# SeanNaren/deepspeech.pytorch

Hardware: NVIDIA H100
Metric: utterances/sec (train step, 161x1000 spectrogram) (higher is better)
Workload: dtype fp16-operands(rnn)+tf32(conv/fc)

## Files before the change

### deepspeech.pytorch_b200/csrc/common.cuh

```cuda
#pragma once
#include <cuda_runtime.h>
#include <stdint.h>
#include <stdio.h>
#include <string.h>
#include <atomic>

#include "../../include/ds2_b200.h"

namespace ds2 {

void set_error(const char* fmt, ...);
extern std::atomic<long long> g_launches;
int precision();
inline bool tensor_core_mode() { return precision() != DS2_PREC_FP32; }
inline bool f16_gemm_mode() { return precision() == DS2_PREC_F16; }

inline cudaStream_t as_stream(void* s) { return reinterpret_cast<cudaStream_t>(s); }

inline int current_device() {
  int d = 0;
  (void)cudaGetDevice(&d);
  return d & 63;
}
struct DeviceOnce {
// ... 62 lines not shown

#ifdef __CUDACC__
__device__ __forceinline__ float sigmoidf_(float x) { return 1.0f / (1.0f + expf(-x)); }

__device__ __forceinline__ float warp_sum(float v) {
#pragma unroll
  for (int o = 16; o > 0; o >>= 1) v += __shfl_xor_sync(0xffffffffu, v, o);
  return v;
}
__device__ __forceinline__ double warp_sum_d(double v) {
#pragma unroll
  for (int o = 16; o > 0; o >>= 1) v += __shfl_xor_sync(0xffffffffu, v, o);
  return v;
}
#endif

int gemm_simt(int transA, int transB, int M, int N, int K, float alpha, const float* A, int lda, const float* B,
              int ldb, float beta, float* C, int ldc, cudaStream_t st, void* ws = nullptr, size_t ws_bytes = 0);
size_t gemm_simt_workspace_bytes(int M, int N, int K);
int gemm_tc(int transA, int transB, int M, int N, int K, float alpha, const float* A, int lda, const float* B,
            int ldb, float beta, float* C, int ldc, void* ws, size_t ws_bytes, cudaStream_t st);
size_t gemm_tc_workspace_bytes(int transA, int transB, int M, int N, int K);
int gemm_tc_f16(int M, int N, int K, float alpha, const void* A16, int lda, const void* B16, int ldb, float beta,
                float* C, int ldc, const float* alpha_dev, cudaStream_t st);
int f32_to_f16_rows(int rows, int cols, const float* in, size_t ld_in, void* out, size_t ld_out, const float* scale_dev,
                    cudaStream_t st);
int f32_to_f16_transpose(int rows, int cols, const float* in, size_t ld_in, void* out, size_t ld_out, void* outT,
                         size_t ld_outT, const float* scale_dev, cudaStream_t st);
int pow2_scale_for(int rows, int cols, const float* x, size_t ld, unsigned int* absmax_ws, float* scale, int top,
                   cudaStream_t st);

int bn_rows_fwd(int rows, int F, const float* x, const float* gamma, const float* beta, float* rmean, float* rvar,
                int training, float momentum, float eps, float* y, float* xhat, float* mean_invstd ,
                double* ws_sums , cudaStream_t st);
int bn_rows_reapply(int rows, int F, const float* x, const float* gamma, const float* beta,
                    const float* mean_invstd, float* y, float* xhat, cudaStream_t st);
int transpose(int R, int C, const float* in, float* out, cudaStream_t st);
int transpose_strided(int R, int C, const float* in, size_t ldi, float* out, size_t ldo, cudaStream_t st);
int bn_rows_bwd(int rows, int F, const float* xhat, const float* gamma, const float* mean_invstd, const float* dy,
                float* dx, float* dgamma, float* dbeta, double* ws_sums , cudaStream_t st);

}
```

### deepspeech.pytorch_b200/csrc/gemm_tc.cu

```cuda
#include <stdio.h>

#include "common.cuh"
#include "tc_common.cuh"

namespace ds2 {

typedef CUresult (*EncodeTiledFn)(CUtensorMap*, CUtensorMapDataType, cuuint32_t, void*, const cuuint64_t*,
                                  const cuuint64_t*, const cuuint32_t*, const cuuint32_t*, CUtensorMapInterleave,
                                  CUtensorMapSwizzle, CUtensorMapL2promotion, CUtensorMapFloatOOBfill);
static EncodeTiledFn g_encode = nullptr;
static constexpr CUtensorMapDataType g_tmap_dtype = CU_TENSOR_MAP_DATA_TYPE_TFLOAT32;

static int load_encode() {
  if (g_encode) return DS2_OK;
  void* fn = nullptr;
  cudaDriverEntryPointQueryResult q;
  DS2_CHECK_CUDA(cudaGetDriverEntryPoint("cuTensorMapEncodeTiled", &fn, cudaEnableDefault, &q));
  if (!fn || q != cudaDriverEntryPointSuccess) {
    set_error("cuTensorMapEncodeTiled not available from the driver");
    return DS2_ERR_CUDA;
  }
  g_encode = reinterpret_cast<EncodeTiledFn>(fn);
  return DS2_OK;
}

static int make_tmap_2d_sw(CUtensorMap* out, const float* base, int rows, int cols, int ld, int box_rows, int box_cols,
                           CUtensorMapSwizzle sw);
int make_tmap_2d(CUtensorMap* out, const float* base, int rows, int cols, int ld, int box_rows, int box_cols) {
  return make_tmap_2d_sw(out, base, rows, cols, ld, box_rows, box_cols, CU_TENSOR_MAP_SWIZZLE_128B);
}
static int make_tmap_2d_sw(CUtensorMap* out, const float* base, int rows, int cols, int ld, int box_rows, int box_cols,
                           CUtensorMapSwizzle sw) {
  int rc = load_encode();
  if (rc) return rc;
  cuuint64_t gdim[2] = {(cuuint64_t)cols, (cuuint64_t)rows};
  cuuint64_t gstr[1] = {(cuuint64_t)ld * sizeof(float)};
  cuuint32_t box[2] = {(cuuint32_t)box_cols, (cuuint32_t)box_rows};
  cuuint32_t estr[2] = {1, 1};
  CUresult r = g_encode(out, g_tmap_dtype, 2, const_cast<float*>(base), gdim, gstr, box, estr,
                        CU_TENSOR_MAP_INTERLEAVE_NONE, sw, CU_TENSOR_MAP_L2_PROMOTION_L2_256B,
                        CU_TENSOR_MAP_FLOAT_OOB_FILL_NONE);
  if (r != CUDA_SUCCESS) {
    set_error("cuTensorMapEncodeTiled(2d rows=%d cols=%d ld=%d box=%dx%d base=%p) failed: %d", rows, cols, ld,
              box_rows, box_cols, (const void*)base, (int)r);
    return DS2_ERR_CUDA;
  }
  return DS2_OK;
}

static int make_tmap_3d_sw(CUtensorMap* out, const float* base, int d0, int d1, int d2, size_t stride1, size_t stride2,
                           int box0, int box1, int box2, CUtensorMapSwizzle sw);
int make_tmap_3d(CUtensorMap* out, const float* base, int d0, int d1, int d2, size_t stride1, size_t stride2,
                 int box0, int box1, int box2) {
  return make_tmap_3d_sw(out, base, d0, d1, d2, stride1, stride2, box0, box1, box2, CU_TENSOR_MAP_SWIZZLE_128B);
}
static int make_tmap_3d_sw(CUtensorMap* out, const float* base, int d0, int d1, int d2, size_t stride1, size_t stride2,
                           int box0, int box1, int box2, CUtensorMapSwizzle sw) {
  int rc = load_encode();
  if (rc) return rc;
  cuuint64_t gdim[3] = {(cuuint64_t)d0, (cuuint64_t)d1, (cuuint64_t)d2};
  cuuint64_t gstr[2] = {(cuuint64_t)stride1 * sizeof(float), (cuuint64_t)stride2 * sizeof(float)};
  cuuint32_t box[3] = {(cuuint32_t)box0, (cuuint32_t)box1, (cuuint32_t)box2};
// ... 53 lines not shown
  cuuint32_t box[3] = {(cuuint32_t)box0, (cuuint32_t)box1, (cuuint32_t)box2};
  cuuint32_t estr[3] = {1, 1, 1};
  CUresult r = g_encode(out, CU_TENSOR_MAP_DATA_TYPE_FLOAT16, (cuuint32_t)rank, const_cast<void*>(base), gdim, gstr,
                        box, estr, CU_TENSOR_MAP_INTERLEAVE_NONE, CU_TENSOR_MAP_SWIZZLE_128B,
                        CU_TENSOR_MAP_L2_PROMOTION_L2_256B, CU_TENSOR_MAP_FLOAT_OOB_FILL_NONE);
  if (r != CUDA_SUCCESS) {
    set_error("cuTensorMapEncodeTiled(f16 rank %d dims %d,%d,%d box %d,%d,%d) failed: %d", rank, d0, d1, d2, box0, box1,
              box2, (int)r);
    return DS2_ERR_CUDA;
  }
  return DS2_OK;
}

namespace gtc {
constexpr int BM = 128, BK = 32, THREADS = 384;
constexpr int PRODUCER_REGS = 40, MMA_REGS = 232;
template <int BN>
struct Cfg {
  static constexpr int STAGES = BN == 256 ? 4 : 6;
  static constexpr int A_BYTES = BM * 128, B_BYTES = BN * 128, STAGE_BYTES = A_BYTES + B_BYTES;
  static constexpr int SMEM_BYTES = STAGES * STAGE_BYTES + 1024  + 256 ;
};
static_assert(Cfg<256>::SMEM_BYTES <= 227 * 1024 && Cfg<128>::SMEM_BYTES <= 227 * 1024, "shared memory");
}

template <bool F16, int BN>
__global__ void __launch_bounds__(gtc::THREADS, 1)
gemm_tc_kernel(const __grid_constant__ CUtensorMap tmA, const __grid_constant__ CUtensorMap tmB, int M, int N, int K,
               float alpha, float beta, float* __restrict__ C, int ldc, const float* __restrict__ alpha_dev) {
  using namespace gtc;
  using namespace tc;
  constexpr int STAGES = Cfg<BN>::STAGES, A_BYTES = Cfg<BN>::A_BYTES, STAGE_BYTES = Cfg<BN>::STAGE_BYTES;
  constexpr int BK = F16 ? 2 * gtc::BK : gtc::BK;
  if (alpha_dev) alpha *= __ldg(alpha_dev);
  extern __shared__ uint8_t smem_raw[];
  uint8_t* smem = smem_raw + ((1024u - (smem_u32(smem_raw) & 1023u)) & 1023u);
  uint64_t* full = reinterpret_cast<uint64_t*>(smem + STAGES * STAGE_BYTES);
  uint64_t* empty = full + STAGES;
  const int warp = threadIdx.x / 32, lane = threadIdx.x % 32;
  const int m0 = blockIdx.y * BM, n0 = blockIdx.x * BN;
  const int nk = (K + BK - 1) / BK;

  if (warp == 0 && lane == 0) {
    tma_prefetch_desc(&tmA);
    tma_prefetch_desc(&tmB);
    for (int i = 0; i < STAGES; ++i) { mbar_init(&full[i], 1); mbar_init(&empty[i], 2); }
// ... 49 lines not shown
        float2 o = make_float2(alpha * acc[4 * i + 2 * hh], alpha * acc[4 * i + 2 * hh + 1]);
        if (vec_ok && col + 1 < N) {
          float2* cp2 = reinterpret_cast<float2*>(crow + col);
          if (beta != 0.f) {
            const float2 old = *cp2;
            o.x = fmaf(beta, old.x, o.x);
            o.y = fmaf(beta, old.y, o.y);
          }
          *cp2 = o;
        } else {
#pragma unroll
          for (int j = 0; j < 2; ++j) {
            if (col + j >= N) break;
            float v = j ? o.y : o.x;
            if (beta != 0.f) v = fmaf(beta, crow[col + j], v);
            crow[col + j] = v;
          }
        }
      }
    }
  }
}

__global__ void transpose_strided_kernel(int R, int C, const float* __restrict__ in, size_t ldi,
                                         float* __restrict__ out, size_t ldo) {
  __shared__ float tile[32][33];
  int c = blockIdx.x * 32 + threadIdx.x, r0 = blockIdx.y * 32;
  for (int j = threadIdx.y; j < 32; j += 8)
    if (r0 + j < R && c < C) tile[j][threadIdx.x] = in[(size_t)(r0 + j) * ldi + c];
  __syncthreads();
  int r = r0 + threadIdx.x, c0 = blockIdx.x * 32;
  for (int j = threadIdx.y; j < 32; j += 8)
    if (c0 + j < C && r < R) out[(size_t)(c0 + j) * ldo + r] = tile[threadIdx.x][j];
}

int transpose_strided(int R, int C, const float* in, size_t ldi, float* out, size_t ldo, cudaStream_t st) {
  DS2_LAUNCH(transpose_strided_kernel, dim3(cdiv(C, 32), cdiv(R, 32)), dim3(32, 8), 0, st, R, C, in, ldi, out, ldo);
  return DS2_OK;
}
int transpose(int R, int C, const float* in, float* out, cudaStream_t st) {
  return transpose_strided(R, C, in, (size_t)C, out, (size_t)R, st);
}

static inline size_t k4(int K) { return (size_t)((K + 3) / 4 * 4); }

struct GemmTcWs { float *At, *Bt; };
static size_t gemm_tc_ws_carve(int transA, int transB, int M, int N, int K, void* base, GemmTcWs& w) {
  size_t off = 0;
  w.At = transA ? carve<float>(base, off, (size_t)M * k4(K) * 4) : nullptr;
  w.Bt = transB ? nullptr : carve<float>(base, off, (size_t)N * k4(K) * 4);
  return off;
}

size_t gemm_tc_workspace_bytes(int transA, int transB, int M, int N, int K) {
  GemmTcWs w;
  return gemm_tc_ws_carve(transA, transB, M, N, K, nullptr, w);
}

static bool tc_eligible(int M, int N, int K) { return K >= 32 && M >= 32 && N >= 16 && (long long)M * N * K >= (1 << 18); }

static int tile_n(int N) { return N > 128 ? 256 : 128; }

template <bool F16, int BN>
static int launch_gemm_tc(const CUtensorMap& tmA, const CUtensorMap& tmB, int M, int N, int K, float alpha, float beta,
                          float* C, int ldc, cudaStream_t st, const float* alpha_dev) {
  auto kern = gemm_tc_kernel<F16, BN>;
  constexpr int smem = gtc::Cfg<BN>::SMEM_BYTES;
  static DeviceOnce attr_once;
  if (attr_once.first()) {
    DS2_CHECK_CUDA(cudaFuncSetAttribute(kern, cudaFuncAttributeMaxDynamicSharedMemorySize, smem));
    attr_once.done();
  }
  dim3 grid(cdiv(N, BN), cdiv(M, gtc::BM));
  DS2_LAUNCH(kern, grid, gtc::THREADS, smem, st, tmA, tmB, M, N, K, alpha, beta, C, ldc, alpha_dev);
  return DS2_OK;
}

template <bool F16>
static int launch_gemm_tc(const CUtensorMap& tmA, const CUtensorMap& tmB, int M, int N, int K, float alpha, float beta,
                          float* C, int ldc, cudaStream_t st, const float* alpha_dev = nullptr) {
  if (tile_n(N) == 256) return launch_gemm_tc<F16, 256>(tmA, tmB, M, N, K, alpha, beta, C, ldc, st, alpha_dev);
  return launch_gemm_tc<F16, 128>(tmA, tmB, M, N, K, alpha, beta, C, ldc, st, alpha_dev);
}

int gemm_tc(int transA, int transB, int M, int N, int K, float alpha, const float* A, int lda, const float* B,
            int ldb, float beta, float* C, int ldc, void* ws, size_t ws_bytes, cudaStream_t st) {
  if (!tc_eligible(M, N, K)) return 1;
  GemmTcWs W;
  if (gemm_tc_ws_carve(transA, transB, M, N, K, ws, W) > (ws ? ws_bytes : 0)) return 1;
  const float* Ak = A;
  int ldak = lda;
  if (transA) {
    int rc = transpose_strided(K, M, A, (size_t)lda, W.At, k4(K), st);
    if (rc) return rc;
    Ak = W.At;
    ldak = (int)k4(K);
  }
  const float* Bk = B;
  int ldbk = ldb;
  if (!transB) {
    int rc = transpose_strided(K, N, B, (size_t)ldb, W.Bt, k4(K), st);
    if (rc) return rc;
    Bk = W.Bt;
    ldbk = (int)k4(K);
  }
  if ((ldak & 3) || (ldbk & 3) || (reinterpret_cast<uintptr_t>(Ak) & 15) || (reinterpret_cast<uintptr_t>(Bk) & 15))
    return 1;
  CUtensorMap tmA, tmB;
  int rc = make_tmap_2d(&tmA, Ak, M, K, ldak, gtc::BM, gtc::BK);
  if (rc) return rc;
  rc = make_tmap_2d(&tmB, Bk, N, K, ldbk, tile_n(N), gtc::BK);
  if (rc) return rc;
  return launch_gemm_tc<false>(tmA, tmB, M, N, K, alpha, beta, C, ldc, st);
}

int gemm_tc_f16(int M, int N, int K, float alpha, const void* A16, int lda, const void* B16, int ldb, float beta,
                float* C, int ldc, const float* alpha_dev, cudaStream_t st) {
  if (!tc_eligible(M, N, K) || M < 128) return 1;
  if ((lda & 7) || (ldb & 7) || (reinterpret_cast<uintptr_t>(A16) & 15) || (reinterpret_cast<uintptr_t>(B16) & 15)) return 1;
  CUtensorMap tmA, tmB;
  int rc = make_tmap_f16(&tmA, A16, 2, K, M, 1, (size_t)lda, 0, 64, gtc::BM, 1);
  if (rc) return rc;
  rc = make_tmap_f16(&tmB, B16, 2, K, N, 1, (size_t)ldb, 0, 64, tile_n(N), 1);
  if (rc) return rc;
  return launch_gemm_tc<true>(tmA, tmB, M, N, K, alpha, beta, C, ldc, st, alpha_dev);
}

}
```

### deepspeech.pytorch_b200/csrc/rnn_layer.cu

```cuda
#include <cuda_fp16.h>

#include <mutex>
#include <unordered_set>

#include "common.cuh"
#include "rnn_cells.cuh"
#include "rnn_common.cuh"

namespace ds2 {

constexpr int UT = 8;
constexpr int KC = 64;

template <int RNN>
__global__ void __launch_bounds__(32 * UT) rnn_step_fwd_kernel(SeqArgs a, int step) {
  constexpr int G = num_gates(RNN);
  __shared__ float hs[32][KC + 1];
  __shared__ float ws[G * UT][KC + 1];
  const int d = blockIdx.y, T = a.T, B = a.B, H = a.H, D = a.D;
  const int t = d == 0 ? step : T - 1 - step;
  const int tp = d == 0 ? t - 1 : t + 1;
  const bool tp_in = tp >= 0 && tp < T;
  const int lane = threadIdx.x, uy = threadIdx.y, tid = uy * 32 + lane;
  const int u0 = blockIdx.x * UT, u = u0 + uy;
// ... 490 lines not shown
  if (f16 && side && d->deferred_dw) {
    rc = side_fork(st, side);
    if (rc) return rc;
    gst = side;
  }
  if (f16) {
    rc = f32_to_f16_transpose(TB, In, xin, (size_t)In, nullptr, 0, W.x16T, (size_t)TB, nullptr, gst);
    if (rc) return rc;
    for (int dir = 0; dir < D; ++dir) {
      rc = f32_to_f16_transpose(TB, H, R.hseq + (size_t)dir * TB * H, (size_t)H, nullptr, 0, W.h16T + (size_t)dir * H * TB,
                                (size_t)TB, nullptr, gst);
      if (rc) return rc;
      if (gru && !made.f16) {
        rc = f32_to_f16_transpose(TB, H, R.aux + (size_t)dir * TB * H, (size_t)H, nullptr, 0,
                                  W.aux16T + (size_t)dir * H * TB, (size_t)TB, W.scale, gst);
        if (rc) return rc;
      }
    }
  }
  auto weight_grad = [&](int M, int N, int K, const __half* A16, const __half* B16, const float* A, int lda,
                         const float* Bf, int ldb, float* C, int ldc) {
    int r = 1;
    if (f16) {
      r = gemm_tc_f16(M, N, K, 1.f, A16, TB, B16, TB, 0.f, C, ldc, W.scale + 1, gst);
      if (r < 0) return r;
    }
    return r == 1 ? ds2_gemm(1, 0, M, N, K, 1.f, A, lda, Bf, ldb, 0.f, C, ldc, gws, gws_bytes, stream) : r;
  };
  auto f16_at = [&](const __half* p, size_t off) { return f16 ? p + off : nullptr; };
  bool dx_done = false;
  if (f16 && dx) {
    rc = gemm_tc_f16(TB, In, D * GH, 1.f, W.dG16, D * GH, W.w16T, D * GH, 0.f, bn_gamma ? W.dxbn : dx, In, W.scale + 1,
                     st);
    if (rc < 0) return rc;
    dx_done = rc == 0;
  }
  for (int dir = 0; dir < D; ++dir) {
    const float* dG = R.gates + (size_t)dir * GH;
    const int ldg = D * GH;
    const float* aux_d = R.aux ? R.aux + (size_t)dir * TB * H : nullptr;
    const float* hseq_d = R.hseq + (size_t)dir * TB * H;
    rc = weight_grad(GH, In, TB, f16_at(W.dG16T, (size_t)dir * GH * TB), W.x16T, dG, ldg, xin, In, dw_ih[dir], In);
    if (rc) return rc;
    if (!made.dbias) {
      rc = colsum(TB, GH, dG, ldg, db_ih[dir], st);
      if (rc) return rc;
    }
// ... 46 lines not shown
```

### deepspeech.pytorch_b200/csrc/tc_common.cuh

```cuda
#pragma once
#include <cuda.h>
#include <cuda_runtime.h>
#include <stdint.h>

#include <type_traits>

#include "wgmma.cuh"

namespace ds2 {
namespace tc {

__device__ __forceinline__ uint32_t smem_u32(const void* p) { return (uint32_t)__cvta_generic_to_shared(p); }

__device__ __forceinline__ void mbar_init(uint64_t* bar, uint32_t count) {
  asm volatile("mbarrier.init.shared::cta.b64 [%0], %1;" ::"r"(smem_u32(bar)), "r"(count));
}
__device__ __forceinline__ void fence_barrier_init() { asm volatile("fence.mbarrier_init.release.cluster;" ::: "memory"); }
__device__ __forceinline__ void fence_proxy_async() { asm volatile("fence.proxy.async.shared::cta;" ::: "memory"); }
__device__ __forceinline__ void mbar_arrive_expect_tx(uint64_t* bar, uint32_t bytes) {
  asm volatile("mbarrier.arrive.expect_tx.shared::cta.b64 _, [%0], %1;" ::"r"(smem_u32(bar)), "r"(bytes) : "memory");
}
__device__ __forceinline__ void mbar_arrive(uint64_t* bar) {
  asm volatile("mbarrier.arrive.shared::cta.b64 _, [%0];" ::"r"(smem_u32(bar)) : "memory");
}
// ... 20 lines not shown
  return ok != 0;
}
__device__ __forceinline__ void mbar_wait(uint64_t* bar, uint32_t parity) {
  while (!mbar_try_wait(bar, parity)) {
  }
}

__device__ __forceinline__ void tma_prefetch_desc(const CUtensorMap* m) {
  asm volatile("prefetch.tensormap [%0];" ::"l"(reinterpret_cast<uint64_t>(m)) : "memory");
}
__device__ __forceinline__ void tma_load_2d(void* smem_dst, const CUtensorMap* m, uint64_t* bar, int c0, int c1) {
  asm volatile(
      "cp.async.bulk.tensor.2d.shared::cluster.global.tile.mbarrier::complete_tx::bytes [%0], [%1, {%3, %4}], [%2];"
      ::"r"(smem_u32(smem_dst)), "l"(reinterpret_cast<uint64_t>(m)), "r"(smem_u32(bar)), "r"(c0), "r"(c1)
      : "memory");
}
__device__ __forceinline__ void tma_load_3d(void* smem_dst, const CUtensorMap* m, uint64_t* bar, int c0, int c1,
                                            int c2) {
  asm volatile(
      "cp.async.bulk.tensor.3d.shared::cluster.global.tile.mbarrier::complete_tx::bytes [%0], [%1, {%3, %4, %5}], [%2];"
      ::"r"(smem_u32(smem_dst)), "l"(reinterpret_cast<uint64_t>(m)), "r"(smem_u32(bar)), "r"(c0), "r"(c1), "r"(c2)
      : "memory");
}

__device__ __forceinline__ void mbar_arrive_expect_tx_w(uint64_t* bar, uint32_t bytes) {
  asm volatile(
      "{\n\t.reg .pred pe;\n\telect.sync _|pe, 0xffffffff;\n\t"
      "@pe mbarrier.arrive.expect_tx.shared::cta.b64 _, [%0], %1;\n\t}" ::"r"(smem_u32(bar)), "r"(bytes)
      : "memory");
}
__device__ __forceinline__ void tma_load_2d_w(void* smem_dst, const CUtensorMap* m, uint64_t* bar, int c0, int c1) {
  asm volatile(
      "{\n\t.reg .pred pe;\n\telect.sync _|pe, 0xffffffff;\n\t"
      "@pe cp.async.bulk.tensor.2d.shared::cluster.global.tile.mbarrier::complete_tx::bytes [%0], [%1, {%3, %4}], [%2];\n\t}"
      ::"r"(smem_u32(smem_dst)), "l"(reinterpret_cast<uint64_t>(m)), "r"(smem_u32(bar)), "r"(c0), "r"(c1)
      : "memory");
}
__device__ __forceinline__ void tma_load_3d_w(void* smem_dst, const CUtensorMap* m, uint64_t* bar, int c0, int c1,
                                              int c2) {
  asm volatile(
      "{\n\t.reg .pred pe;\n\telect.sync _|pe, 0xffffffff;\n\t"
      "@pe cp.async.bulk.tensor.3d.shared::cluster.global.tile.mbarrier::complete_tx::bytes [%0], [%1, {%3, %4, %5}], [%2];\n\t}"
      ::"r"(smem_u32(smem_dst)), "l"(reinterpret_cast<uint64_t>(m)), "r"(smem_u32(bar)), "r"(c0), "r"(c1), "r"(c2)
      : "memory");
}

// ... 110 lines not shown
```

### deepspeech.pytorch_b200/csrc/wgmma.cuh

```cuda
#pragma once
#include <stdint.h>

namespace ds2 {
namespace tc {

template <int N, bool F16>
struct Wgmma;

template <>
struct Wgmma<8, false> {
  __device__ __forceinline__ static void mma(float* d, uint64_t a, uint64_t b, uint32_t acc) {
    asm volatile(
        "{\n\t.reg .pred p;\n\tsetp.ne.b32 p, %6, 0;\n\t"
        "wgmma.mma_async.sync.aligned.m64n8k8.f32.tf32.tf32 {%0, %1, %2, %3}, %4, %5, p, 1, 1;\n\t}"
        : "+f"(d[0]), "+f"(d[1]), "+f"(d[2]), "+f"(d[3])
        : "l"(a), "l"(b), "r"(acc));
  }
};

template <>
struct Wgmma<8, true> {
  __device__ __forceinline__ static void mma(float* d, uint64_t a, uint64_t b, uint32_t acc) {
    asm volatile(
        "{\n\t.reg .pred p;\n\tsetp.ne.b32 p, %6, 0;\n\t"
// ... 116 lines not shown
template <>
struct Wgmma<176, false> {
  __device__ __forceinline__ static void mma(float* d, uint64_t a, uint64_t b, uint32_t acc) {
    asm volatile(
        "{\n\t.reg .pred p;\n\tsetp.ne.b32 p, %90, 0;\n\t"
        "wgmma.mma_async.sync.aligned.m64n176k8.f32.tf32.tf32 {%0, %1, %2, %3, %4, %5, %6, %7, %8, %9, %10, %11, %12, %13, %14, %15, %16, %17, %18, %19, %20, %21, %22, %23, %24, %25, %26, %27, %28, %29, %30, %31, %32, %33, %34, %35, %36, %37, %38, %39, %40, %41, %42, %43, %44, %45, %46, %47, %48, %49, %50, %51, %52, %53, %54, %55, %56, %57, %58, %59, %60, %61, %62, %63, %64, %65, %66, %67, %68, %69, %70, %71, %72, %73, %74, %75, %76, %77, %78, %79, %80, %81, %82, %83, %84, %85, %86, %87}, %88, %89, p, 1, 1;\n\t}"
        : "+f"(d[0]), "+f"(d[1]), "+f"(d[2]), "+f"(d[3]), "+f"(d[4]), "+f"(d[5]), "+f"(d[6]), "+f"(d[7]), "+f"(d[8]), "+f"(d[9]), "+f"(d[10]), "+f"(d[11]), "+f"(d[12]), "+f"(d[13]), "+f"(d[14]), "+f"(d[15]), "+f"(d[16]), "+f"(d[17]), "+f"(d[18]), "+f"(d[19]), "+f"(d[20]), "+f"(d[21]), "+f"(d[22]), "+f"(d[23]), "+f"(d[24]), "+f"(d[25]), "+f"(d[26]), "+f"(d[27]), "+f"(d[28]), "+f"(d[29]), "+f"(d[30]), "+f"(d[31]), "+f"(d[32]), "+f"(d[33]), "+f"(d[34]), "+f"(d[35]), "+f"(d[36]), "+f"(d[37]), "+f"(d[38]), "+f"(d[39]), "+f"(d[40]), "+f"(d[41]), "+f"(d[42]), "+f"(d[43]), "+f"(d[44]), "+f"(d[45]), "+f"(d[46]), "+f"(d[47]), "+f"(d[48]), "+f"(d[49]), "+f"(d[50]), "+f"(d[51]), "+f"(d[52]), "+f"(d[53]), "+f"(d[54]), "+f"(d[55]), "+f"(d[56]), "+f"(d[57]), "+f"(d[58]), "+f"(d[59]), "+f"(d[60]), "+f"(d[61]), "+f"(d[62]), "+f"(d[63]), "+f"(d[64]), "+f"(d[65]), "+f"(d[66]), "+f"(d[67]), "+f"(d[68]), "+f"(d[69]), "+f"(d[70]), "+f"(d[71]), "+f"(d[72]), "+f"(d[73]), "+f"(d[74]), "+f"(d[75]), "+f"(d[76]), "+f"(d[77]), "+f"(d[78]), "+f"(d[79]), "+f"(d[80]), "+f"(d[81]), "+f"(d[82]), "+f"(d[83]), "+f"(d[84]), "+f"(d[85]), "+f"(d[86]), "+f"(d[87])
        : "l"(a), "l"(b), "r"(acc));
  }
};

template <>
struct Wgmma<176, true> {
  __device__ __forceinline__ static void mma(float* d, uint64_t a, uint64_t b, uint32_t acc) {
    asm volatile(
        "{\n\t.reg .pred p;\n\tsetp.ne.b32 p, %90, 0;\n\t"
        "wgmma.mma_async.sync.aligned.m64n176k16.f32.f16.f16 {%0, %1, %2, %3, %4, %5, %6, %7, %8, %9, %10, %11, %12, %13, %14, %15, %16, %17, %18, %19, %20, %21, %22, %23, %24, %25, %26, %27, %28, %29, %30, %31, %32, %33, %34, %35, %36, %37, %38, %39, %40, %41, %42, %43, %44, %45, %46, %47, %48, %49, %50, %51, %52, %53, %54, %55, %56, %57, %58, %59, %60, %61, %62, %63, %64, %65, %66, %67, %68, %69, %70, %71, %72, %73, %74, %75, %76, %77, %78, %79, %80, %81, %82, %83, %84, %85, %86, %87}, %88, %89, p, 1, 1, 0, 0;\n\t}"
        : "+f"(d[0]), "+f"(d[1]), "+f"(d[2]), "+f"(d[3]), "+f"(d[4]), "+f"(d[5]), "+f"(d[6]), "+f"(d[7]), "+f"(d[8]), "+f"(d[9]), "+f"(d[10]), "+f"(d[11]), "+f"(d[12]), "+f"(d[13]), "+f"(d[14]), "+f"(d[15]), "+f"(d[16]), "+f"(d[17]), "+f"(d[18]), "+f"(d[19]), "+f"(d[20]), "+f"(d[21]), "+f"(d[22]), "+f"(d[23]), "+f"(d[24]), "+f"(d[25]), "+f"(d[26]), "+f"(d[27]), "+f"(d[28]), "+f"(d[29]), "+f"(d[30]), "+f"(d[31]), "+f"(d[32]), "+f"(d[33]), "+f"(d[34]), "+f"(d[35]), "+f"(d[36]), "+f"(d[37]), "+f"(d[38]), "+f"(d[39]), "+f"(d[40]), "+f"(d[41]), "+f"(d[42]), "+f"(d[43]), "+f"(d[44]), "+f"(d[45]), "+f"(d[46]), "+f"(d[47]), "+f"(d[48]), "+f"(d[49]), "+f"(d[50]), "+f"(d[51]), "+f"(d[52]), "+f"(d[53]), "+f"(d[54]), "+f"(d[55]), "+f"(d[56]), "+f"(d[57]), "+f"(d[58]), "+f"(d[59]), "+f"(d[60]), "+f"(d[61]), "+f"(d[62]), "+f"(d[63]), "+f"(d[64]), "+f"(d[65]), "+f"(d[66]), "+f"(d[67]), "+f"(d[68]), "+f"(d[69]), "+f"(d[70]), "+f"(d[71]), "+f"(d[72]), "+f"(d[73]), "+f"(d[74]), "+f"(d[75]), "+f"(d[76]), "+f"(d[77]), "+f"(d[78]), "+f"(d[79]), "+f"(d[80]), "+f"(d[81]), "+f"(d[82]), "+f"(d[83]), "+f"(d[84]), "+f"(d[85]), "+f"(d[86]), "+f"(d[87])
        : "l"(a), "l"(b), "r"(acc));
  }
};

template <>
struct Wgmma<256, false> {
  __device__ __forceinline__ static void mma(float* d, uint64_t a, uint64_t b, uint32_t acc) {
    asm volatile(
        "{\n\t.reg .pred p;\n\tsetp.ne.b32 p, %130, 0;\n\t"
        "wgmma.mma_async.sync.aligned.m64n256k8.f32.tf32.tf32 {%0, %1, %2, %3, %4, %5, %6, %7, %8, %9, %10, %11, %12, %13, %14, %15, %16, %17, %18, %19, %20, %21, %22, %23, %24, %25, %26, %27, %28, %29, %30, %31, %32, %33, %34, %35, %36, %37, %38, %39, %40, %41, %42, %43, %44, %45, %46, %47, %48, %49, %50, %51, %52, %53, %54, %55, %56, %57, %58, %59, %60, %61, %62, %63, %64, %65, %66, %67, %68, %69, %70, %71, %72, %73, %74, %75, %76, %77, %78, %79, %80, %81, %82, %83, %84, %85, %86, %87, %88, %89, %90, %91, %92, %93, %94, %95, %96, %97, %98, %99, %100, %101, %102, %103, %104, %105, %106, %107, %108, %109, %110, %111, %112, %113, %114, %115, %116, %117, %118, %119, %120, %121, %122, %123, %124, %125, %126, %127}, %128, %129, p, 1, 1;\n\t}"
        : "+f"(d[0]), "+f"(d[1]), "+f"(d[2]), "+f"(d[3]), "+f"(d[4]), "+f"(d[5]), "+f"(d[6]), "+f"(d[7]), "+f"(d[8]), "+f"(d[9]), "+f"(d[10]), "+f"(d[11]), "+f"(d[12]), "+f"(d[13]), "+f"(d[14]), "+f"(d[15]), "+f"(d[16]), "+f"(d[17]), "+f"(d[18]), "+f"(d[19]), "+f"(d[20]), "+f"(d[21]), "+f"(d[22]), "+f"(d[23]), "+f"(d[24]), "+f"(d[25]), "+f"(d[26]), "+f"(d[27]), "+f"(d[28]), "+f"(d[29]), "+f"(d[30]), "+f"(d[31]), "+f"(d[32]), "+f"(d[33]), "+f"(d[34]), "+f"(d[35]), "+f"(d[36]), "+f"(d[37]), "+f"(d[38]), "+f"(d[39]), "+f"(d[40]), "+f"(d[41]), "+f"(d[42]), "+f"(d[43]), "+f"(d[44]), "+f"(d[45]), "+f"(d[46]), "+f"(d[47]), "+f"(d[48]), "+f"(d[49]), "+f"(d[50]), "+f"(d[51]), "+f"(d[52]), "+f"(d[53]), "+f"(d[54]), "+f"(d[55]), "+f"(d[56]), "+f"(d[57]), "+f"(d[58]), "+f"(d[59]), "+f"(d[60]), "+f"(d[61]), "+f"(d[62]), "+f"(d[63]), "+f"(d[64]), "+f"(d[65]), "+f"(d[66]), "+f"(d[67]), "+f"(d[68]), "+f"(d[69]), "+f"(d[70]), "+f"(d[71]), "+f"(d[72]), "+f"(d[73]), "+f"(d[74]), "+f"(d[75]), "+f"(d[76]), "+f"(d[77]), "+f"(d[78]), "+f"(d[79]), "+f"(d[80]), "+f"(d[81]), "+f"(d[82]), "+f"(d[83]), "+f"(d[84]), "+f"(d[85]), "+f"(d[86]), "+f"(d[87]), "+f"(d[88]), "+f"(d[89]), "+f"(d[90]), "+f"(d[91]), "+f"(d[92]), "+f"(d[93]), "+f"(d[94]), "+f"(d[95]), "+f"(d[96]), "+f"(d[97]), "+f"(d[98]), "+f"(d[99]), "+f"(d[100]), "+f"(d[101]), "+f"(d[102]), "+f"(d[103]), "+f"(d[104]), "+f"(d[105]), "+f"(d[106]), "+f"(d[107]), "+f"(d[108]), "+f"(d[109]), "+f"(d[110]), "+f"(d[111]), "+f"(d[112]), "+f"(d[113]), "+f"(d[114]), "+f"(d[115]), "+f"(d[116]), "+f"(d[117]), "+f"(d[118]), "+f"(d[119]), "+f"(d[120]), "+f"(d[121]), "+f"(d[122]), "+f"(d[123]), "+f"(d[124]), "+f"(d[125]), "+f"(d[126]), "+f"(d[127])
        : "l"(a), "l"(b), "r"(acc));
  }
};

template <>
struct Wgmma<256, true> {
  __device__ __forceinline__ static void mma(float* d, uint64_t a, uint64_t b, uint32_t acc) {
    asm volatile(
        "{\n\t.reg .pred p;\n\tsetp.ne.b32 p, %130, 0;\n\t"
        "wgmma.mma_async.sync.aligned.m64n256k16.f32.f16.f16 {%0, %1, %2, %3, %4, %5, %6, %7, %8, %9, %10, %11, %12, %13, %14, %15, %16, %17, %18, %19, %20, %21, %22, %23, %24, %25, %26, %27, %28, %29, %30, %31, %32, %33, %34, %35, %36, %37, %38, %39, %40, %41, %42, %43, %44, %45, %46, %47, %48, %49, %50, %51, %52, %53, %54, %55, %56, %57, %58, %59, %60, %61, %62, %63, %64, %65, %66, %67, %68, %69, %70, %71, %72, %73, %74, %75, %76, %77, %78, %79, %80, %81, %82, %83, %84, %85, %86, %87, %88, %89, %90, %91, %92, %93, %94, %95, %96, %97, %98, %99, %100, %101, %102, %103, %104, %105, %106, %107, %108, %109, %110, %111, %112, %113, %114, %115, %116, %117, %118, %119, %120, %121, %122, %123, %124, %125, %126, %127}, %128, %129, p, 1, 1, 0, 0;\n\t}"
        : "+f"(d[0]), "+f"(d[1]), "+f"(d[2]), "+f"(d[3]), "+f"(d[4]), "+f"(d[5]), "+f"(d[6]), "+f"(d[7]), "+f"(d[8]), "+f"(d[9]), "+f"(d[10]), "+f"(d[11]), "+f"(d[12]), "+f"(d[13]), "+f"(d[14]), "+f"(d[15]), "+f"(d[16]), "+f"(d[17]), "+f"(d[18]), "+f"(d[19]), "+f"(d[20]), "+f"(d[21]), "+f"(d[22]), "+f"(d[23]), "+f"(d[24]), "+f"(d[25]), "+f"(d[26]), "+f"(d[27]), "+f"(d[28]), "+f"(d[29]), "+f"(d[30]), "+f"(d[31]), "+f"(d[32]), "+f"(d[33]), "+f"(d[34]), "+f"(d[35]), "+f"(d[36]), "+f"(d[37]), "+f"(d[38]), "+f"(d[39]), "+f"(d[40]), "+f"(d[41]), "+f"(d[42]), "+f"(d[43]), "+f"(d[44]), "+f"(d[45]), "+f"(d[46]), "+f"(d[47]), "+f"(d[48]), "+f"(d[49]), "+f"(d[50]), "+f"(d[51]), "+f"(d[52]), "+f"(d[53]), "+f"(d[54]), "+f"(d[55]), "+f"(d[56]), "+f"(d[57]), "+f"(d[58]), "+f"(d[59]), "+f"(d[60]), "+f"(d[61]), "+f"(d[62]), "+f"(d[63]), "+f"(d[64]), "+f"(d[65]), "+f"(d[66]), "+f"(d[67]), "+f"(d[68]), "+f"(d[69]), "+f"(d[70]), "+f"(d[71]), "+f"(d[72]), "+f"(d[73]), "+f"(d[74]), "+f"(d[75]), "+f"(d[76]), "+f"(d[77]), "+f"(d[78]), "+f"(d[79]), "+f"(d[80]), "+f"(d[81]), "+f"(d[82]), "+f"(d[83]), "+f"(d[84]), "+f"(d[85]), "+f"(d[86]), "+f"(d[87]), "+f"(d[88]), "+f"(d[89]), "+f"(d[90]), "+f"(d[91]), "+f"(d[92]), "+f"(d[93]), "+f"(d[94]), "+f"(d[95]), "+f"(d[96]), "+f"(d[97]), "+f"(d[98]), "+f"(d[99]), "+f"(d[100]), "+f"(d[101]), "+f"(d[102]), "+f"(d[103]), "+f"(d[104]), "+f"(d[105]), "+f"(d[106]), "+f"(d[107]), "+f"(d[108]), "+f"(d[109]), "+f"(d[110]), "+f"(d[111]), "+f"(d[112]), "+f"(d[113]), "+f"(d[114]), "+f"(d[115]), "+f"(d[116]), "+f"(d[117]), "+f"(d[118]), "+f"(d[119]), "+f"(d[120]), "+f"(d[121]), "+f"(d[122]), "+f"(d[123]), "+f"(d[124]), "+f"(d[125]), "+f"(d[126]), "+f"(d[127])
        : "l"(a), "l"(b), "r"(acc));
  }
};

}
}
// ... 1 lines not shown
```

Before: 659.3.

## Add persistent TMA-store GEMM kernel with N=224 tiles for beta-zero outputs

Adds a persistent warp-specialized WGMMA GEMM whose tiles stride over the grid, with the epilogue staged through swizzled shared memory and written back by TMA bulk stores. When beta is zero and C is aligned, the planner picks BN=224 if that yields the same tile count as 256, so less of each tile is wasted on padding. The goal is to cut launch and tail overhead and make the epilogue stores cheaper. Persistence is turned off when the RNN GEMM runs on a side stream, so it does not claim every SM while other work runs alongside it. Risks include a non-overlapped epilogue per tile and the smaller k-ring that the staging buffers leave room for.

```diff
diff --git a/deepspeech.pytorch_b200/csrc/common.cuh b/deepspeech.pytorch_b200/csrc/common.cuh
--- a/deepspeech.pytorch_b200/csrc/common.cuh
+++ b/deepspeech.pytorch_b200/csrc/common.cuh
@@ -108,7 +108,7 @@
             int ldb, float beta, float* C, int ldc, void* ws, size_t ws_bytes, cudaStream_t st);
 size_t gemm_tc_workspace_bytes(int transA, int transB, int M, int N, int K);
 int gemm_tc_f16(int M, int N, int K, float alpha, const void* A16, int lda, const void* B16, int ldb, float beta,
-                float* C, int ldc, const float* alpha_dev, cudaStream_t st);
+                float* C, int ldc, const float* alpha_dev, cudaStream_t st, bool persistent = true);
 int f32_to_f16_rows(int rows, int cols, const float* in, size_t ld_in, void* out, size_t ld_out, const float* scale_dev,
                     cudaStream_t st);
 int f32_to_f16_transpose(int rows, int cols, const float* in, size_t ld_in, void* out, size_t ld_out, void* outT,
diff --git a/deepspeech.pytorch_b200/csrc/gemm_tc.cu b/deepspeech.pytorch_b200/csrc/gemm_tc.cu
--- a/deepspeech.pytorch_b200/csrc/gemm_tc.cu
+++ b/deepspeech.pytorch_b200/csrc/gemm_tc.cu
@@ -25,19 +25,19 @@
 }
 
 static int make_tmap_2d_sw(CUtensorMap* out, const float* base, int rows, int cols, int ld, int box_rows, int box_cols,
-                           CUtensorMapSwizzle sw);
+                           CUtensorMapSwizzle sw, CUtensorMapDataType dtype = g_tmap_dtype);
 int make_tmap_2d(CUtensorMap* out, const float* base, int rows, int cols, int ld, int box_rows, int box_cols) {
   return make_tmap_2d_sw(out, base, rows, cols, ld, box_rows, box_cols, CU_TENSOR_MAP_SWIZZLE_128B);
 }
 static int make_tmap_2d_sw(CUtensorMap* out, const float* base, int rows, int cols, int ld, int box_rows, int box_cols,
-                           CUtensorMapSwizzle sw) {
+                           CUtensorMapSwizzle sw, CUtensorMapDataType dtype) {
   int rc = load_encode();
   if (rc) return rc;
   cuuint64_t gdim[2] = {(cuuint64_t)cols, (cuuint64_t)rows};
   cuuint64_t gstr[1] = {(cuuint64_t)ld * sizeof(float)};
   cuuint32_t box[2] = {(cuuint32_t)box_cols, (cuuint32_t)box_rows};
   cuuint32_t estr[2] = {1, 1};
-  CUresult r = g_encode(out, g_tmap_dtype, 2, const_cast<float*>(base), gdim, gstr, box, estr,
+  CUresult r = g_encode(out, dtype, 2, const_cast<float*>(base), gdim, gstr, box, estr,
                         CU_TENSOR_MAP_INTERLEAVE_NONE, sw, CU_TENSOR_MAP_L2_PROMOTION_L2_256B,
                         CU_TENSOR_MAP_FLOAT_OOB_FILL_NONE);
   if (r != CUDA_SUCCESS) {
@@ -137,6 +137,15 @@
   static constexpr int SMEM_BYTES = STAGES * STAGE_BYTES + 1024  + 256 ;
 };
 static_assert(Cfg<256>::SMEM_BYTES <= 227 * 1024 && Cfg<128>::SMEM_BYTES <= 227 * 1024, "shared memory");
+template <int BN>
+struct StoreCfg {
+  static constexpr int STAGES = 4, SBUF = BN == 256 ? 2 : 3;
+  static constexpr int A_BYTES = BM * 128, B_BYTES = BN * 128, STAGE_BYTES = A_BYTES + B_BYTES;
+  static constexpr int RING_BYTES = STAGES * STAGE_BYTES, SUB_BYTES = 64 * 128;
+  static constexpr int SMEM_BYTES = RING_BYTES + 2 * SBUF * SUB_BYTES + 1024  + 256 ;
+  static_assert(STAGE_BYTES % 1024 == 0, "stages stay 1024-byte aligned for the 128-byte swizzle");
+};
+static_assert(StoreCfg<256>::SMEM_BYTES <= 227 * 1024 && StoreCfg<224>::SMEM_BYTES <= 227 * 1024, "shared memory");
 }
 
 template <bool F16, int BN>
@@ -232,6 +241,105 @@
   }
 }
 
+template <bool F16, int BN>
+__global__ void __launch_bounds__(gtc::THREADS, 1)
+gemm_tc_persistent_kernel(const __grid_constant__ CUtensorMap tmA, const __grid_constant__ CUtensorMap tmB,
+                          const __grid_constant__ CUtensorMap tmC, int M, int N, int K, float alpha,
+                          const float* __restrict__ alpha_dev) {
+  using namespace gtc;
+  using namespace tc;
+  using Cf = StoreCfg<BN>;
+  constexpr int STAGES = Cf::STAGES, SBUF = Cf::SBUF, A_BYTES = Cf::A_BYTES, STAGE_BYTES = Cf::STAGE_BYTES;
+  constexpr int BK = F16 ? 2 * gtc::BK : gtc::BK;
+  if (alpha_dev) alpha *= __ldg(alpha_dev);
+  extern __shared__ uint8_t smem_raw[];
+  uint8_t* smem = smem_raw + ((1024u - (smem_u32(smem_raw) & 1023u)) & 1023u);
+  uint8_t* staging = smem + Cf::RING_BYTES;
+  uint64_t* full = reinterpret_cast<uint64_t*>(staging + 2 * SBUF * Cf::SUB_BYTES);
+  uint64_t* empty = full + STAGES;
+  const int warp = threadIdx.x / 32, lane = threadIdx.x % 32;
+  const int nk = (K + BK - 1) / BK, tiles_n = (N + BN - 1) / BN, tiles = (M + BM - 1) / BM * tiles_n;
+
+  if (warp == 0 && lane == 0) {
+    tma_prefetch_desc(&tmA);
+    tma_prefetch_desc(&tmB);
+    tma_prefetch_desc(&tmC);
+    for (int i = 0; i < STAGES; ++i) { mbar_init(&full[i], 1); mbar_init(&empty[i], 2); }
+    fence_barrier_init();
+  }
+  __syncthreads();
+
+  if (warp < 4) {
+    setmaxnreg_dec<PRODUCER_REGS>();
+    if (warp == 0 && lane == 0) {
+      int it = 0;
+      for (int t = blockIdx.x; t < tiles; t += gridDim.x) {
+        const int m0 = t / tiles_n * BM, n0 = t % tiles_n * BN;
+        for (int kt = 0; kt < nk; ++kt, ++it) {
+          const int s = it % STAGES;
+          mbar_wait(&empty[s], ((it / STAGES) & 1) ^ 1);
+          mbar_arrive_expect_tx(&full[s], STAGE_BYTES);
+          uint8_t* sa = smem + s * STAGE_BYTES;
+          tma_load_2d(sa, &tmA, &full[s], kt * BK, m0);
+          tma_load_2d(sa + A_BYTES, &tmB, &full[s], kt * BK, n0);
+        }
+      }
+    }
+  } else {
+    setmaxnreg_inc<MMA_REGS>();
+    const int wg = warp / 4 - 1, w = warp % 4;
+    const bool leader = (threadIdx.x & 127) == 0;
+    uint8_t* out = staging + wg * SBUF * Cf::SUB_BYTES;
+    int it = 0, sub = 0;
+    for (int t = blockIdx.x; t < tiles; t += gridDim.x) {
+      const int m0 = t / tiles_n * BM, n0 = t % tiles_n * BN;
+      float acc[BN / 2];
+#pragma unroll
+      for (int i = 0; i < BN / 2; ++i) acc[i] = 0.f;
+      for (int kt = 0; kt < nk; ++kt, ++it) {
+        const int s = it % STAGES;
+        mbar_wait(&full[s], (it / STAGES) & 1);
+        const uint64_t adesc = smem_desc_sw128(smem_u32(smem + s * STAGE_BYTES)) + (uint64_t)(512 * wg);
+        const uint64_t bdesc = smem_desc_sw128(smem_u32(smem + s * STAGE_BYTES + A_BYTES));
+        wg_fence();
+#pragma unroll
+        for (int k = 0; k < 4; ++k)
+          Wgmma<BN, F16>::mma(acc, adesc + 2 * k, bdesc + 2 * k, 1u);
+        wg_commit();
+        wg_wait<1>();
+        if (kt > 0 && leader) mbar_arrive(&empty[(it - 1) % STAGES]);
+      }
+      wg_wait<0>();
+      if (leader) mbar_arrive(&empty[(it - 1) % STAGES]);
+      const bool rows_in = m0 + 64 * wg < M;
+#pragma unroll
+      for (int c = 0; c < BN / 32; ++c) {
+        if (!rows_in || n0 + 32 * c >= N) continue;
+        uint8_t* buf = out + (sub++ % SBUF) * Cf::SUB_BYTES;
+        if (leader) bulk_wait_read<SBUF - 1>();
+        asm volatile("bar.sync %0, 128;" ::"r"(1 + wg) : "memory");
+#pragma unroll
+        for (int i = 0; i < 4; ++i) {
+#pragma unroll
+          for (int hh = 0; hh < 2; ++hh) {
+            const int r = 16 * w + (lane >> 2) + 8 * hh, chunk = 2 * i + ((lane & 3) >> 1);
+            const int a = 4 * (4 * c + i) + 2 * hh;
+            *reinterpret_cast<float2*>(buf + r * 128 + ((chunk ^ (r & 7)) << 4) + ((lane & 1) << 3)) =
+                make_float2(alpha * acc[a], alpha * acc[a + 1]);
+          }
+        }
+        fence_proxy_async();
+        asm volatile("bar.sync %0, 128;" ::"r"(1 + wg) : "memory");
+        if (leader) {
+          tma_store_2d(&tmC, buf, n0 + 32 * c, m0 + 64 * wg);
+          bulk_commit();
+        }
+      }
+    }
+    if (leader) bulk_wait<0>();
+  }
+}
+
 __global__ void transpose_strided_kernel(int R, int C, const float* __restrict__ in, size_t ldi,
                                          float* __restrict__ out, size_t ldo) {
   __shared__ float tile[32][33];
@@ -269,7 +377,15 @@
 
 static bool tc_eligible(int M, int N, int K) { return K >= 32 && M >= 32 && N >= 16 && (long long)M * N * K >= (1 << 18); }
 
-static int tile_n(int N) { return N > 128 ? 256 : 128; }
+struct TilePlan {
+  int bn;
+  bool store;
+};
+static TilePlan plan_tiles(int N, float beta, const float* C, int ldc) {
+  if (N <= 128) return {128, false};
+  if (beta != 0.f || (ldc & 3) || (reinterpret_cast<uintptr_t>(C) & 15)) return {256, false};
+  return {cdiv(N, 224) == cdiv(N, 256) ? 224 : 256, true};
+}
 
 template <bool F16, int BN>
 static int launch_gemm_tc(const CUtensorMap& tmA, const CUtensorMap& tmB, int M, int N, int K, float alpha, float beta,
@@ -286,10 +402,33 @@
   return DS2_OK;
 }
 
+template <bool F16, int BN>
+static int launch_gemm_tc_persistent(const CUtensorMap& tmA, const CUtensorMap& tmB, int M, int N, int K, float alpha,
+                                     float* C, int ldc, cudaStream_t st, const float* alpha_dev, bool persistent) {
+  CUtensorMap tmC;
+  int rc = make_tmap_2d_sw(&tmC, C, M, N, ldc, 64, 32, CU_TENSOR_MAP_SWIZZLE_128B, CU_TENSOR_MAP_DATA_TYPE_FLOAT32);
+  if (rc) return rc;
+  auto kern = gemm_tc_persistent_kernel<F16, BN>;
+  constexpr int smem = gtc::StoreCfg<BN>::SMEM_BYTES;
+  static DeviceOnce attr_once;
+  if (attr_once.first()) {
+    DS2_CHECK_CUDA(cudaFuncSetAttribute(kern, cudaFuncAttributeMaxDynamicSharedMemorySize, smem));
+    attr_once.done();
+  }
+  const int tiles = cdiv(M, gtc::BM) * cdiv(N, BN);
+  const int grid = persistent && tiles > device_sm_count() ? device_sm_count() : tiles;
+  DS2_LAUNCH(kern, grid, gtc::THREADS, smem, st, tmA, tmB, tmC, M, N, K, alpha, alpha_dev);
+  return DS2_OK;
+}
+
 template <bool F16>
-static int launch_gemm_tc(const CUtensorMap& tmA, const CUtensorMap& tmB, int M, int N, int K, float alpha, float beta,
-                          float* C, int ldc, cudaStream_t st, const float* alpha_dev = nullptr) {
-  if (tile_n(N) == 256) return launch_gemm_tc<F16, 256>(tmA, tmB, M, N, K, alpha, beta, C, ldc, st, alpha_dev);
+static int launch_gemm_tc(const CUtensorMap& tmA, const CUtensorMap& tmB, TilePlan plan, int M, int N, int K,
+                          float alpha, float beta, float* C, int ldc, cudaStream_t st, const float* alpha_dev,
+                          bool persistent) {
+  if (plan.store && plan.bn == 224)
+    return launch_gemm_tc_persistent<F16, 224>(tmA, tmB, M, N, K, alpha, C, ldc, st, alpha_dev, persistent);
+  if (plan.store) return launch_gemm_tc_persistent<F16, 256>(tmA, tmB, M, N, K, alpha, C, ldc, st, alpha_dev, persistent);
+  if (plan.bn == 256) return launch_gemm_tc<F16, 256>(tmA, tmB, M, N, K, alpha, beta, C, ldc, st, alpha_dev);
   return launch_gemm_tc<F16, 128>(tmA, tmB, M, N, K, alpha, beta, C, ldc, st, alpha_dev);
 }
 
@@ -316,24 +455,26 @@
   }
   if ((ldak & 3) || (ldbk & 3) || (reinterpret_cast<uintptr_t>(Ak) & 15) || (reinterpret_cast<uintptr_t>(Bk) & 15))
     return 1;
+  const TilePlan plan = plan_tiles(N, beta, C, ldc);
   CUtensorMap tmA, tmB;
   int rc = make_tmap_2d(&tmA, Ak, M, K, ldak, gtc::BM, gtc::BK);
   if (rc) return rc;
-  rc = make_tmap_2d(&tmB, Bk, N, K, ldbk, tile_n(N), gtc::BK);
-  if (rc) return rc;
-  return launch_gemm_tc<false>(tmA, tmB, M, N, K, alpha, beta, C, ldc, st);
+  rc = make_tmap_2d(&tmB, Bk, N, K, ldbk, plan.bn, gtc::BK);
+  if (rc) return rc;
+  return launch_gemm_tc<false>(tmA, tmB, plan, M, N, K, alpha, beta, C, ldc, st, nullptr, true);
 }
 
 int gemm_tc_f16(int M, int N, int K, float alpha, const void* A16, int lda, const void* B16, int ldb, float beta,
-                float* C, int ldc, const float* alpha_dev, cudaStream_t st) {
+                float* C, int ldc, const float* alpha_dev, cudaStream_t st, bool persistent) {
   if (!tc_eligible(M, N, K) || M < 128) return 1;
   if ((lda & 7) || (ldb & 7) || (reinterpret_cast<uintptr_t>(A16) & 15) || (reinterpret_cast<uintptr_t>(B16) & 15)) return 1;
+  const TilePlan plan = plan_tiles(N, beta, C, ldc);
   CUtensorMap tmA, tmB;
   int rc = make_tmap_f16(&tmA, A16, 2, K, M, 1, (size_t)lda, 0, 64, gtc::BM, 1);
   if (rc) return rc;
-  rc = make_tmap_f16(&tmB, B16, 2, K, N, 1, (size_t)ldb, 0, 64, tile_n(N), 1);
-  if (rc) return rc;
-  return launch_gemm_tc<true>(tmA, tmB, M, N, K, alpha, beta, C, ldc, st, alpha_dev);
-}
-
-}
+  rc = make_tmap_f16(&tmB, B16, 2, K, N, 1, (size_t)ldb, 0, 64, plan.bn, 1);
+  if (rc) return rc;
+  return launch_gemm_tc<true>(tmA, tmB, plan, M, N, K, alpha, beta, C, ldc, st, alpha_dev, persistent);
+}
+
+}
diff --git a/deepspeech.pytorch_b200/csrc/rnn_layer.cu b/deepspeech.pytorch_b200/csrc/rnn_layer.cu
--- a/deepspeech.pytorch_b200/csrc/rnn_layer.cu
+++ b/deepspeech.pytorch_b200/csrc/rnn_layer.cu
@@ -536,7 +536,7 @@
                          const float* Bf, int ldb, float* C, int ldc) {
     int r = 1;
     if (f16) {
-      r = gemm_tc_f16(M, N, K, 1.f, A16, TB, B16, TB, 0.f, C, ldc, W.scale + 1, gst);
+      r = gemm_tc_f16(M, N, K, 1.f, A16, TB, B16, TB, 0.f, C, ldc, W.scale + 1, gst, gst == st);
       if (r < 0) return r;
     }
     return r == 1 ? ds2_gemm(1, 0, M, N, K, 1.f, A, lda, Bf, ldb, 0.f, C, ldc, gws, gws_bytes, stream) : r;
diff --git a/deepspeech.pytorch_b200/csrc/tc_common.cuh b/deepspeech.pytorch_b200/csrc/tc_common.cuh
--- a/deepspeech.pytorch_b200/csrc/tc_common.cuh
+++ b/deepspeech.pytorch_b200/csrc/tc_common.cuh
@@ -66,6 +66,17 @@
       ::"r"(smem_u32(smem_dst)), "l"(reinterpret_cast<uint64_t>(m)), "r"(smem_u32(bar)), "r"(c0), "r"(c1), "r"(c2)
       : "memory");
 }
+
+__device__ __forceinline__ void tma_store_2d(const CUtensorMap* m, const void* smem_src, int c0, int c1) {
+  asm volatile("cp.async.bulk.tensor.2d.global.shared::cta.bulk_group [%0, {%2, %3}], [%1];"
+               ::"l"(reinterpret_cast<uint64_t>(m)), "r"(smem_u32(smem_src)), "r"(c0), "r"(c1)
+               : "memory");
+}
+__device__ __forceinline__ void bulk_commit() { asm volatile("cp.async.bulk.commit_group;" ::: "memory"); }
+template <int N>
+__device__ __forceinline__ void bulk_wait_read() { asm volatile("cp.async.bulk.wait_group.read %0;" ::"n"(N) : "memory"); }
+template <int N>
+__device__ __forceinline__ void bulk_wait() { asm volatile("cp.async.bulk.wait_group %0;" ::"n"(N) : "memory"); }
 
 __device__ __forceinline__ void mbar_arrive_expect_tx_w(uint64_t* bar, uint32_t bytes) {
   asm volatile(
diff --git a/deepspeech.pytorch_b200/csrc/wgmma.cuh b/deepspeech.pytorch_b200/csrc/wgmma.cuh
--- a/deepspeech.pytorch_b200/csrc/wgmma.cuh
+++ b/deepspeech.pytorch_b200/csrc/wgmma.cuh
@@ -162,6 +162,28 @@
 };
 
 template <>
+struct Wgmma<224, false> {
+  __device__ __forceinline__ static void mma(float* d, uint64_t a, uint64_t b, uint32_t acc) {
+    asm volatile(
+        "{\n\t.reg .pred p;\n\tsetp.ne.b32 p, %114, 0;\n\t"
+        "wgmma.mma_async.sync.aligned.m64n224k8.f32.tf32.tf32 {%0, %1, %2, %3, %4, %5, %6, %7, %8, %9, %10, %11, %12, %13, %14, %15, %16, %17, %18, %19, %20, %21, %22, %23, %24, %25, %26, %27, %28, %29, %30, %31, %32, %33, %34, %35, %36, %37, %38, %39, %40, %41, %42, %43, %44, %45, %46, %47, %48, %49, %50, %51, %52, %53, %54, %55, %56, %57, %58, %59, %60, %61, %62, %63, %64, %65, %66, %67, %68, %69, %70, %71, %72, %73, %74, %75, %76, %77, %78, %79, %80, %81, %82, %83, %84, %85, %86, %87, %88, %89, %90, %91, %92, %93, %94, %95, %96, %97, %98, %99, %100, %101, %102, %103, %104, %105, %106, %107, %108, %109, %110, %111}, %112, %113, p, 1, 1;\n\t}"
+        : "+f"(d[0]), "+f"(d[1]), "+f"(d[2]), "+f"(d[3]), "+f"(d[4]), "+f"(d[5]), "+f"(d[6]), "+f"(d[7]), "+f"(d[8]), "+f"(d[9]), "+f"(d[10]), "+f"(d[11]), "+f"(d[12]), "+f"(d[13]), "+f"(d[14]), "+f"(d[15]), "+f"(d[16]), "+f"(d[17]), "+f"(d[18]), "+f"(d[19]), "+f"(d[20]), "+f"(d[21]), "+f"(d[22]), "+f"(d[23]), "+f"(d[24]), "+f"(d[25]), "+f"(d[26]), "+f"(d[27]), "+f"(d[28]), "+f"(d[29]), "+f"(d[30]), "+f"(d[31]), "+f"(d[32]), "+f"(d[33]), "+f"(d[34]), "+f"(d[35]), "+f"(d[36]), "+f"(d[37]), "+f"(d[38]), "+f"(d[39]), "+f"(d[40]), "+f"(d[41]), "+f"(d[42]), "+f"(d[43]), "+f"(d[44]), "+f"(d[45]), "+f"(d[46]), "+f"(d[47]), "+f"(d[48]), "+f"(d[49]), "+f"(d[50]), "+f"(d[51]), "+f"(d[52]), "+f"(d[53]), "+f"(d[54]), "+f"(d[55]), "+f"(d[56]), "+f"(d[57]), "+f"(d[58]), "+f"(d[59]), "+f"(d[60]), "+f"(d[61]), "+f"(d[62]), "+f"(d[63]), "+f"(d[64]), "+f"(d[65]), "+f"(d[66]), "+f"(d[67]), "+f"(d[68]), "+f"(d[69]), "+f"(d[70]), "+f"(d[71]), "+f"(d[72]), "+f"(d[73]), "+f"(d[74]), "+f"(d[75]), "+f"(d[76]), "+f"(d[77]), "+f"(d[78]), "+f"(d[79]), "+f"(d[80]), "+f"(d[81]), "+f"(d[82]), "+f"(d[83]), "+f"(d[84]), "+f"(d[85]), "+f"(d[86]), "+f"(d[87]), "+f"(d[88]), "+f"(d[89]), "+f"(d[90]), "+f"(d[91]), "+f"(d[92]), "+f"(d[93]), "+f"(d[94]), "+f"(d[95]), "+f"(d[96]), "+f"(d[97]), "+f"(d[98]), "+f"(d[99]), "+f"(d[100]), "+f"(d[101]), "+f"(d[102]), "+f"(d[103]), "+f"(d[104]), "+f"(d[105]), "+f"(d[106]), "+f"(d[107]), "+f"(d[108]), "+f"(d[109]), "+f"(d[110]), "+f"(d[111])
+        : "l"(a), "l"(b), "r"(acc));
+  }
+};
+
+template <>
+struct Wgmma<224, true> {
+  __device__ __forceinline__ static void mma(float* d, uint64_t a, uint64_t b, uint32_t acc) {
+    asm volatile(
+        "{\n\t.reg .pred p;\n\tsetp.ne.b32 p, %114, 0;\n\t"
+        "wgmma.mma_async.sync.aligned.m64n224k16.f32.f16.f16 {%0, %1, %2, %3, %4, %5, %6, %7, %8, %9, %10, %11, %12, %13, %14, %15, %16, %17, %18, %19, %20, %21, %22, %23, %24, %25, %26, %27, %28, %29, %30, %31, %32, %33, %34, %35, %36, %37, %38, %39, %40, %41, %42, %43, %44, %45, %46, %47, %48, %49, %50, %51, %52, %53, %54, %55, %56, %57, %58, %59, %60, %61, %62, %63, %64, %65, %66, %67, %68, %69, %70, %71, %72, %73, %74, %75, %76, %77, %78, %79, %80, %81, %82, %83, %84, %85, %86, %87, %88, %89, %90, %91, %92, %93, %94, %95, %96, %97, %98, %99, %100, %101, %102, %103, %104, %105, %106, %107, %108, %109, %110, %111}, %112, %113, p, 1, 1, 0, 0;\n\t}"
+        : "+f"(d[0]), "+f"(d[1]), "+f"(d[2]), "+f"(d[3]), "+f"(d[4]), "+f"(d[5]), "+f"(d[6]), "+f"(d[7]), "+f"(d[8]), "+f"(d[9]), "+f"(d[10]), "+f"(d[11]), "+f"(d[12]), "+f"(d[13]), "+f"(d[14]), "+f"(d[15]), "+f"(d[16]), "+f"(d[17]), "+f"(d[18]), "+f"(d[19]), "+f"(d[20]), "+f"(d[21]), "+f"(d[22]), "+f"(d[23]), "+f"(d[24]), "+f"(d[25]), "+f"(d[26]), "+f"(d[27]), "+f"(d[28]), "+f"(d[29]), "+f"(d[30]), "+f"(d[31]), "+f"(d[32]), "+f"(d[33]), "+f"(d[34]), "+f"(d[35]), "+f"(d[36]), "+f"(d[37]), "+f"(d[38]), "+f"(d[39]), "+f"(d[40]), "+f"(d[41]), "+f"(d[42]), "+f"(d[43]), "+f"(d[44]), "+f"(d[45]), "+f"(d[46]), "+f"(d[47]), "+f"(d[48]), "+f"(d[49]), "+f"(d[50]), "+f"(d[51]), "+f"(d[52]), "+f"(d[53]), "+f"(d[54]), "+f"(d[55]), "+f"(d[56]), "+f"(d[57]), "+f"(d[58]), "+f"(d[59]), "+f"(d[60]), "+f"(d[61]), "+f"(d[62]), "+f"(d[63]), "+f"(d[64]), "+f"(d[65]), "+f"(d[66]), "+f"(d[67]), "+f"(d[68]), "+f"(d[69]), "+f"(d[70]), "+f"(d[71]), "+f"(d[72]), "+f"(d[73]), "+f"(d[74]), "+f"(d[75]), "+f"(d[76]), "+f"(d[77]), "+f"(d[78]), "+f"(d[79]), "+f"(d[80]), "+f"(d[81]), "+f"(d[82]), "+f"(d[83]), "+f"(d[84]), "+f"(d[85]), "+f"(d[86]), "+f"(d[87]), "+f"(d[88]), "+f"(d[89]), "+f"(d[90]), "+f"(d[91]), "+f"(d[92]), "+f"(d[93]), "+f"(d[94]), "+f"(d[95]), "+f"(d[96]), "+f"(d[97]), "+f"(d[98]), "+f"(d[99]), "+f"(d[100]), "+f"(d[101]), "+f"(d[102]), "+f"(d[103]), "+f"(d[104]), "+f"(d[105]), "+f"(d[106]), "+f"(d[107]), "+f"(d[108]), "+f"(d[109]), "+f"(d[110]), "+f"(d[111])
+        : "l"(a), "l"(b), "r"(acc));
+  }
+};
+
+template <>
 struct Wgmma<256, false> {
   __device__ __forceinline__ static void mma(float* d, uint64_t a, uint64_t b, uint32_t acc) {
     asm volatile(
```

After: 666.4, median of 6. +1.1%, better.
